# ShudaLi/rgbd_pose_estimation

Measured on AMD Instinct MI355X. Metric: correspondence-residuals/sec, higher is better.
Workload: dtype f32; 1 GPU; configs[1]: 640x480 dense depth, 307200 3D-3D corr, point-to-point GN step (K1 normal eq + host 6x6 solve + SE3 exp) over inlier mask; corr_rank0=307200, global_corr=307200, collective=none, rccl_ranks=0, rccl_verified=False, repeats=1

## Files before the change

### rgbd_pose_estimation_amd/csrc/rpe_normal_eq.hip

```cpp
#include "rpe_residuals.hpp"

namespace rpe {

__global__ void gn_update_probe_kernel(const double* __restrict__ rec, double* __restrict__ pose, double* __restrict__ step_ok,
                                       double rel_floor) {
  __shared__ double s_rec[32];
  __shared__ double s_pose[12];
  if (threadIdx.x < 32) s_rec[threadIdx.x] = rec[threadIdx.x];
  if (threadIdx.x < 12) s_pose[threadIdx.x] = pose[threadIdx.x];
  __syncthreads();
  if (threadIdx.x == 0) {
    double step = 0.0;
    const bool ok = gn_solve_update<0>(s_rec, s_pose, &step, rel_floor);
    step_ok[0] = step; step_ok[1] = ok ? 1.0 : 0.0;
    if (ok) for (int k = 0; k < 12; k++) pose[k] = s_pose[k];
  }
}
hipError_t launch_gn_update_probe(const double* d_rec, double* d_pose, double* d_step_ok, double pivot_floor, hipStream_t s) {
  hipLaunchKernelGGL(gn_update_probe_kernel, dim3(1), dim3(64), 0, s, d_rec, d_pose, d_step_ok, pivot_floor);
  return hipGetLastError();
}

template <class T, int KIND, int BLK, bool MASK, bool WEIGHT, bool CLEAN>
__global__ __launch_bounds__(BLK) void normal_eq_kernel(const T* __restrict__ xw, const T* __restrict__ b, const T* __restrict__ c,
// ... 65 lines not shown
    if (++carried == kShare) { flush_pairs<T, NACC>(carry, acc); carried = 0; }
    a0 = na0; a1 = na1; a2 = na2; b0 = nb0; b1 = nb1; b2 = nb2;
    if (KIND == KIND_P2PLANE) { c0 = nc0; c1 = nc1; c2 = nc2; }
    __builtin_amdgcn_sched_barrier(0);
    pin16(a0); pin16(a1); pin16(a2); pin16(b0); pin16(b1); pin16(b2);
    if (KIND == KIND_P2PLANE) { pin16(c0); pin16(c1); pin16(c2); }
#pragma unroll
    for (int i = 0; i < P; i++) { if (MASK) m[i] = nm[i]; if (WEIGHT) wv[i] = nwv[i]; }
    g = gn;
  }
  if (blockIdx.x == 0 && threadIdx.x == 0 && full * P < n) {
    T vw[3 * P], vb[3 * P], vc[3 * P];
    short lm[P];
    T lwv[P];
    load_group<T>(xw, full, n, vw);
    load_group<T>(b, full, n, vb);
    if (KIND == KIND_P2PLANE) load_group<T>(c, full, n, vc);
    if (MASK) load_scalars<T, short>(mask, full, n, lm, (short)0);
    if (WEIGHT) load_scalars<T, T>(weight, full, n, lwv, T(0));
    pair_group<T, KIND, MASK, WEIGHT, CLEAN, NACC>(pose, vw, vb, vc, lm, lwv, (int)(n - full * P), carry);
    carried = 1;
  }
  if (carried) flush_pairs<T, NACC>(carry, acc);
  RPE_STAMP(1);
  reduce_and_finish<NACC, kNeLd, KIND == KIND_P2P ? 1 : 0, BLK>(acc, fin);
}

template <class T, int KIND, int BLK, bool MASK, bool WEIGHT, int NREG, int AUTO, bool CLEAN>
__global__ __launch_bounds__(BLK) void normal_eq_resident_kernel(const T* __restrict__ xw, const T* __restrict__ b, const T* __restrict__ c,
                             const short* __restrict__ mask, const T* __restrict__ weight, int64_t n,
                             const unsigned long long* __restrict__ ctl, unsigned long long first_tag, int max_iters, Finish fin) {
  constexpr int P = Pk<T>::P;
  constexpr int NACC = KIND == KIND_P2P ? 17 : 29;
  constexpr bool IN_REGS = NREG > 0;
  constexpr int GPT = IN_REGS ? NREG : 1;
  __shared__ double s_pose[12];
  __shared__ int s_go;
  const int64_t full = n / P, groups = (n + P - 1) / P;
  constexpr bool with_solver = AUTO == 2;
  const int workers = (int)gridDim.x;
  const int64_t stride = (int64_t)workers * BLK;
  const int64_t g0 = (int64_t)blockIdx.x * (BLK * GPT) + threadIdx.x;
  T rw[GPT][3 * P], rb[GPT][3 * P], rc[GPT][3 * P];
  short rm[GPT][P];
  T rwv[GPT][P];
  int rpresent[GPT];
#pragma unroll
  for (int r = 0; r < GPT; r++) {
    rpresent[r] = 0;
    const int64_t g = g0 + (int64_t)r * BLK;
    if (IN_REGS && g < groups) {
      load_any_group<T, KIND, MASK, WEIGHT>(xw, b, c, mask, weight, g, full, n, rw[r], rb[r], rc[r], rm[r], rwv[r]);
      rpresent[r] = g < full ? P : (int)(n - full * P);
    }
  }
#ifdef RPE_SOLVER_DEBUG
  if (with_solver && threadIdx.x == 0) __hip_atomic_store(solver_pose_area(fin, workers, NACC) + 32 + blockIdx.x, wall_clock64(), __ATOMIC_RELAXED, __HIP_MEMORY_SCOPE_AGENT);
#endif
  constexpr bool autonomous = AUTO != 0;
  double tol = 0.0;
  if (autonomous) {
    if (threadIdx.x < 12) s_pose[threadIdx.x] = fin.gn_pose[threadIdx.x];
    tol = fin.gn->tol;
    __syncthreads();
  }
  for (int it = 1; it <= max_iters; it++) {
    if (!autonomous && resident_wait_pose<BLK>(ctl, first_tag + (unsigned long long)it, s_pose, &s_go,
        fin.pose_wait_ticks) != 1) return;
    if (with_solver && it > 1 && solver_wait_pose<BLK>(solver_pose_area(fin, workers, NACC), first_tag + (unsigned long long)it, s_pose, &s_go, it == 2 ? kSolverMeetTicks : 200000000ull) != 0) return;
#ifdef RPE_STAMPS
    const bool stamp_it = it == 1000;
    if (stamp_it) RPE_STAMP(0);
#endif
    PoseK<double> pose;
#pragma unroll
    for (int k = 0; k < 9; k++) pose.R[k] = s_pose[k];
#pragma unroll
    for (int k = 0; k < 3; k++) pose.t[k] = s_pose[9 + k];
    double acc[NACC];
#pragma unroll
    for (int k = 0; k < NACC; k++) acc[k] = 0.0;
    if (IN_REGS) {
#pragma unroll
      for (int r = 0; r < GPT; r++)
        if (rpresent[r] > 0) normal_eq_group<T, KIND, MASK, WEIGHT, NACC, CLEAN>(pose, rw[r], rb[r], rc[r], rm[r], rwv[r], rpresent[r], acc);
    } else {
      for (int64_t g = g0; g < groups; g += stride) {
        T vw[3 * P], vb[3 * P], vc[3 * P];
        short mm[P];
        T ww[P];
        load_any_group<T, KIND, MASK, WEIGHT>(xw, b, c, mask, weight, g, full, n, vw, vb, vc, mm, ww);
        normal_eq_group<T, KIND, MASK, WEIGHT, NACC, CLEAN>(pose, vw, vb, vc, mm, ww, g < full ? P : (int)(n - full * P), acc);
      }
    }
#ifdef RPE_STAMPS
    if (stamp_it) RPE_STAMP(1);
#endif
#ifndef RPE_STAMPS
    const bool stamp_it = false;
#endif
    if (with_solver) { solver_send_sums<NACC, BLK>(acc, fin, first_tag + (unsigned long long)it); continue; }
    if (autonomous) {
      if (resident_auto_stage<NACC, BLK>(acc, fin, first_tag + (unsigned long long)it, it, max_iters, tol, s_pose,
          stamp_it) != 0) return;
      continue;
    }
    if (!resident_cross_stage<NACC, BLK>(acc, fin, first_tag + (unsigned long long)it, fin.seq + (unsigned long long)it,
        stamp_it)) return;
  }
}

#ifdef RPE_STAMPS
}
extern "C" int rpe_debug_read_stamps(unsigned long long* out, int nwords) {
  if (nwords > 4096 * 16) nwords = 4096 * 16;
  if (hipDeviceSynchronize() != hipSuccess) return -1;
  if (hipMemcpyFromSymbol(out, HIP_SYMBOL(rpe::g_stamps), (size_t)nwords * 8) != hipSuccess) return -1;
  static unsigned long long zeros[4096 * 16];
  return hipMemcpyToSymbol(HIP_SYMBOL(rpe::g_stamps), zeros, sizeof(zeros)) == hipSuccess ? 0 : -1;
}
namespace rpe {
#endif

template <int MODE>
__global__ __launch_bounds__(64) void chain_finish_kernel(const double* __restrict__ runs, const double* __restrict__ pose_in, GnState* st,
                                                          double rel_floor, double* __restrict__ h_pairs, unsigned long long seq) {
  __shared__ double f_tot[32];
  __shared__ double f_pose[12];
  __shared__ double f_out[16];
  if (threadIdx.x < 12) f_pose[threadIdx.x] = pose_in[threadIdx.x];
  if (threadIdx.x < 32) {
    double t = 0.0;
#pragma unroll
    for (int r = 0; r < kRunSlots; r++) t += runs[r * kRunLd + threadIdx.x];
    f_tot[threadIdx.x] = t;
  }
  __syncthreads();
  if (threadIdx.x == 0) {
    double step = st->step;
    bool ok = st->status == 0;
    if (!st->done) ok = gn_solve_update<MODE>(f_tot, f_pose, &step, rel_floor);
    for (int k = 0; k < 12; k++) f_out[k] = f_pose[k];
    f_out[12] = step; f_out[13] = st->done ? st->cost : record_entry<MODE>(f_tot, 27); f_out[14] = (double)(st->iters + (st->done ? 0 : 1));
    f_out[15] = ok ? 0.0 : 1.0;
  }
  __syncthreads();
  if (threadIdx.x < 16) store_tagged_pair(h_pairs, threadIdx.x, f_out[threadIdx.x], seq);
}
hipError_t launch_chain_finish(int kind, const double* d_runs, const double* d_pose, GnState* d_state, double pivot_floor, double* h_pairs,
                               unsigned long long seq, hipStream_t s) {
  if (kind == KIND_P2P) hipLaunchKernelGGL((chain_finish_kernel<1>), dim3(1), dim3(64), 0, s, d_runs, d_pose, d_state, pivot_floor, h_pairs, seq);
  else hipLaunchKernelGGL((chain_finish_kernel<0>), dim3(1), dim3(64), 0, s, d_runs, d_pose, d_state, pivot_floor, h_pairs, seq);
  return hipGetLastError();
}

template <class T, int KIND, int BLK>
static void normal_eq_launch(const DeviceArrays& A, int flags, const PoseK<double>& pose, const ReduceTarget& rt, hipStream_t s,
                             hipEvent_t ev0, hipEvent_t ev1) {
  const T* xw = (const T*)A.a[0];
  const T* b = (const T*)((KIND == KIND_BEARING || KIND == KIND_REPROJ) ? A.a[2] : A.a[1]);
  const T* c = (const T*)A.a[4];
  const int mod = (KIND == KIND_BEARING || KIND == KIND_REPROJ) ? 0 : 1;
  const short* mask = (flags & F_USE_MASK) ? A.mask[mod] : nullptr;
  const T* weight = (flags & F_USE_WEIGHT) ? (const T*)A.weight[mod] : nullptr;
  const int G = reduce_grid(A.n, Pk<T>::P, rt.max_blocks, BLK);
  const Finish fin = make_finish(rt);
#define RPE_NE_LAUNCH2(M, W, C) RPE_LAUNCH_EV((normal_eq_kernel<T, KIND, BLK, M, W, C>), dim3(G), dim3(BLK), 0, s, ev0, ev1, xw, b, c, mask, weight, A.n, pose, fin)
#define RPE_NE_LAUNCH(M, W) do { if constexpr (sizeof(T) == 4) { if (rt.clean) { RPE_NE_LAUNCH2(M, W, true); break; } } RPE_NE_LAUNCH2(M, W, false); } while (0)
// ... 150 lines not shown
```

### rgbd_pose_estimation_amd/csrc/rpe_reduce.hpp

```cpp
#pragma once
#include "rpe_kernels.h"
#include <cstring>
#include <cstdlib>
#include <algorithm>
#include <hip/hip_ext.h>

namespace rpe {

#ifdef RPE_STAMPS
static __device__ unsigned long long g_stamps[4096 * 16];
#define RPE_STAMP(k)                                                                                             \
  do {                                                                                                           \
    __builtin_amdgcn_sched_barrier(0);                                                                           \
    if (threadIdx.x == 0) {                                                                                      \
      unsigned long long t_;                                                                                     \
      asm volatile("s_memrealtime %0\n\ts_waitcnt lgkmcnt(0)" : "=s"(t_) : : "memory");                          \
      g_stamps[(size_t)blockIdx.x * 16 + (k)] = t_;                                                              \
    }                                                                                                            \
    __builtin_amdgcn_sched_barrier(0);                                                                           \
  } while (0)
#else
#define RPE_STAMP(k) do {} while (0)
#endif

// ... 429 lines not shown
}

template <int NACC, int LD, int BLK, int U>
__device__ __forceinline__ void sum_records(const double* __restrict__ partials, int first, int step, int count, double (*part)[LD],
                                            double* __restrict__ tot) {
  constexpr int RG = BLK / LD;
  const int j = threadIdx.x % LD, rg = threadIdx.x / LD;
  double s = 0.0;
  if (j < NACC) {
    for (int r0 = rg; r0 < count; r0 += RG * U) {
      double v[U];
#pragma unroll
      for (int u = 0; u < U; u++) {
        const int r = r0 + u * RG;
        v[u] = r < count ? __hip_atomic_load(partials + (size_t)(first + r * step) * LD + j, __ATOMIC_RELAXED,
            __HIP_MEMORY_SCOPE_AGENT) : 0.0;
      }
#pragma unroll
      for (int u = 0; u < U; u++) s += v[u];
    }
  }
  part[rg][j] = s;
  __syncthreads();
  if (threadIdx.x < LD) {
    double t = 0.0;
#pragma unroll
    for (int k = 0; k < RG; k++) t += part[k][threadIdx.x];
    tot[threadIdx.x] = threadIdx.x < NACC ? t : 0.0;
  }
}

template <int NACC, int BLK, int CH = 4>
__device__ __forceinline__ bool collect_rows(unsigned long long* __restrict__ gran, int G, int leader, int rows, unsigned long long tag,
                                             double (*part)[NACC], int step = 1,
                                             unsigned long long wait_ticks = 200000000ull) {
  constexpr int RGN = BLK / NACC;
  const int j = threadIdx.x % NACC, r = threadIdx.x / NACC;
  bool lost = false;
  if (CH == 1) {
    if (r >= 1 && r < rows) {
      const unsigned long long* src = gran + 2 * ((size_t)(leader + r * step) * NACC + j);
      const unsigned long long t0 = wall_clock64();
      granule_t q;
      for (unsigned int spins = 1;; spins++) {
        q = load_granule16(src);
        if ((((unsigned long long)q.w << 32) | q.z) == tag) break;
        if ((spins & 63u) == 0 && wall_clock64() - t0 > wait_ticks) { lost = true; break; }
      }
      part[r][j] = __longlong_as_double((long long)(((unsigned long long)q.y << 32) | q.x));
    }
  } else if (r < RGN && r < rows) {
    double sum = r == 0 ? part[0][j] : 0.0;
    const auto rsrc = __builtin_amdgcn_make_buffer_rsrc(reinterpret_cast<void*>(gran), 0, G * NACC * 16, 0x00020000);
    const unsigned long long t0 = wall_clock64();
    for (int k0 = r == 0 ? RGN : r; k0 < rows && !lost; k0 += CH * RGN) {
      granule_t q[CH];
      for (unsigned int spins = 1;; spins++) {
        bool pending = false;
        asm volatile("" ::: "memory");
#pragma unroll
        for (int u = 0; u < CH; u++) {
          const int row = k0 + u * RGN;
          if (row < rows) q[u] = __builtin_amdgcn_raw_buffer_load_b128(rsrc, ((leader + row * step) * NACC + j) * 16, 0, 16);
        }
#pragma unroll
        for (int u = 0; u < CH; u++) {
          const int row = k0 + u * RGN;
          if (row < rows && (((unsigned long long)q[u].w << 32) | q[u].z) != tag) pending = true;
        }
        if (!pending) break;
        if ((spins & 63u) == 0 && wall_clock64() - t0 > wait_ticks) { lost = true; break; }
      }
#pragma unroll
      for (int u = 0; u < CH; u++) {
        const int row = k0 + u * RGN;
        if (row < rows && !lost) sum += __longlong_as_double((long long)(((unsigned long long)q[u].y << 32) | q[u].x));
      }
    }
    part[r][j] = sum;
  }
  return lost;
}

template <int NACC, int RGN>
__device__ __forceinline__ double sum_rows_lane(const double (*part)[NACC], int nr, int j) {
  constexpr int CH = RGN < 16 ? RGN : 16;
  double a = 0.0, b = 0.0;
  for (int k0 = 0; k0 < nr; k0 += CH) {
    double v[CH];
#pragma unroll
    for (int k = 0; k < CH; k++) v[k] = part[k0 + k < RGN ? k0 + k : RGN - 1][j];
#pragma unroll
    for (int k = 0; k < CH; k += 2) {
      a += k0 + k < nr ? v[k] : 0.0;
      if (k + 1 < CH) b += k0 + k + 1 < nr ? v[k + 1] : 0.0;
    }
  }
  return a + b;
}

template <int NACC, int BLK>
__device__ __forceinline__ double sum_rows(const double (*part)[NACC], int nr) {
  constexpr int RGN = BLK / NACC, RB = 6, NB = (RGN + RB - 1) / RB;
  static_assert(NB * NACC <= BLK, "one thread per (block of rows, value)");
  __shared__ double s_blk[NB][NACC];
  const int j = threadIdx.x % NACC, q = threadIdx.x / NACC;
  if (q < NB) {
    double v[RB];
#pragma unroll
    for (int u = 0; u < RB; u++) { const int k = q * RB + u; v[u] = k < nr ? part[k < RGN ? k : 0][j] : 0.0; }
    double t = v[0];
#pragma unroll
    for (int u = 1; u < RB; u++) t += v[u];
    s_blk[q][j] = t;
  }
  __syncthreads();
  double t = 0.0;
  if (threadIdx.x < NACC) {
    t = s_blk[0][threadIdx.x];
#pragma unroll
    for (int b = 1; b < NB; b++) t += s_blk[b][threadIdx.x];
  }
  return t;
}

template <int NACC, int MODE, int BLK>
__device__ __forceinline__ void collect_and_send(const double (*red)[NACC], const Finish& fin) {
  constexpr int NW = BLK / 64;
  constexpr int RGN = BLK / NACC;
  constexpr int kMaxRuns = 512 / NACC > 0 ? 512 / NACC : 1;
  __shared__ double c_part[RGN][NACC];
  unsigned long long* gran = reinterpret_cast<unsigned long long*>(fin.partials);
  const int G = gridDim.x;
  int mult = (G + RGN * 8 - 1) / (RGN * 8);
  if (mult > 4) mult = 4;
  const int mult_cap = (G + RGN * kMaxRuns - 1) / (RGN * kMaxRuns);
  if (mult < mult_cap) mult = mult_cap;
  int R = RGN * mult;
  if (R > fin.rows) R = fin.rows;
  const int S = fin.stride;
  const bool per_xcd = S > 1 && S * NACC <= 512 + NACC && G >= 4 * S && (G + S - 1) / S <= 4 * RGN && (G + S - 1) / S <= fin.rows;
  const int run = per_xcd ? (int)blockIdx.x % S : (int)blockIdx.x / R, leader = per_xcd ? run : run * R, step = per_xcd ? S : 1;
  const int nruns = per_xcd ? S : (G + R - 1) / R;
  if (threadIdx.x < NACC) {
    double own = red[0][threadIdx.x];
#pragma unroll
    for (int w = 1; w < NW; w++) own += red[w][threadIdx.x];
    if ((int)blockIdx.x != leader) store_granule16(gran + 2 * ((size_t)blockIdx.x * NACC + threadIdx.x), own, fin.seq);
    else c_part[0][threadIdx.x] = own;
  }
  RPE_STAMP(4);
  if ((int)blockIdx.x != leader) return;
  const int rows = per_xcd ? (G - run + S - 1) / S : min(R, G - leader);
  const bool lost = collect_rows<NACC, BLK>(gran, G, leader, rows, fin.seq, c_part, step);
  RPE_STAMP(7);
  if (__syncthreads_or(lost)) return;
  RPE_STAMP(8);
  if (fin.out_dev != nullptr) {
    if (threadIdx.x < NACC) fin.out_dev[run * kRunLd + threadIdx.x] = sum_rows_lane<NACC, RGN>(c_part, rows < RGN ? rows : RGN, threadIdx.x);
    if (blockIdx.x == 0) for (int i = nruns * kRunLd + (int)threadIdx.x; i < kRunSlots * kRunLd; i += BLK) fin.out_dev[i] = 0.0;
    return;
  }
  if (threadIdx.x < NACC) store_tagged_pair(fin.out_host, 1 + run * NACC + threadIdx.x,
      sum_rows_lane<NACC, RGN>(c_part, rows < RGN ? rows : RGN, threadIdx.x), fin.seq);
  if (blockIdx.x == 0 && threadIdx.x == 64) {
    const unsigned long long hdr = (unsigned long long)nruns | ((unsigned long long)NACC << 16) | ((unsigned long long)MODE << 24);
    store_tagged_pair(fin.out_host, 0, __longlong_as_double((long long)hdr), fin.seq);
  }
  RPE_STAMP(9);
}

template <int NACC, int LD, int MODE, int BLK, bool GN = true>
__device__ __forceinline__ void reduce_and_finish(double (&acc)[NACC], const Finish& fin) {
  constexpr int NW = BLK / 64;
  constexpr int RG = BLK / LD;
  __shared__ double red[NW][NACC];
  __shared__ double part[RG][LD];
  __shared__ double tot[LD];
  __shared__ int s_last;
  const int lane = threadIdx.x & 63, wave = threadIdx.x >> 6;
  wave_reduce_to<NACC>(acc, red[wave], lane);
  RPE_STAMP(2);
  __syncthreads();
  RPE_STAMP(3);
  if (fin.rows > 0) { collect_and_send<NACC, MODE, BLK>(red, fin); return; }
  const int G = gridDim.x;
  if (G > 1) {
    if (threadIdx.x < NACC) {
      double s = red[0][threadIdx.x];
#pragma unroll
      for (int w = 1; w < NW; w++) s += red[w][threadIdx.x];
      __hip_atomic_store(fin.partials + (size_t)blockIdx.x * LD + threadIdx.x, s, __ATOMIC_RELAXED, __HIP_MEMORY_SCOPE_AGENT);
    }
    asm volatile("s_waitcnt vmcnt(0)" ::: "memory");
    RPE_STAMP(4);
    __syncthreads();
    RPE_STAMP(5);
    const int shard = blockIdx.x & 7;
    const int in_shard = (G - shard + 7) >> 3, shards = G < 8 ? G : 8;
    const int tailv = fin.tail & 3;
    if (tailv != 1) {
      if (threadIdx.x == 0) {
        int last = 0;
        unsigned int* sc = fin.ticket + 32 * shard;
        if (__hip_atomic_fetch_add(sc, 1u, __ATOMIC_RELAXED, __HIP_MEMORY_SCOPE_AGENT) == (unsigned int)in_shard - 1) {
          __hip_atomic_store(sc, 0u, __ATOMIC_RELAXED, __HIP_MEMORY_SCOPE_AGENT);
          unsigned int* top = fin.ticket + 32 * 8;
          if (__hip_atomic_fetch_add(top, 1u, __ATOMIC_RELAXED, __HIP_MEMORY_SCOPE_AGENT) == (unsigned int)shards - 1) {
            __hip_atomic_store(top, 0u, __ATOMIC_RELAXED, __HIP_MEMORY_SCOPE_AGENT);
            last = 1;
          }
        }
        s_last = last;
      }
      RPE_STAMP(6);
      __syncthreads();
      if (!s_last) return;
      RPE_STAMP(7);
      if (tailv == 2) sum_records<NACC, LD, BLK, 16>(fin.partials, 0, 1, G, part, tot);
      else sum_records<NACC, LD, BLK, 8>(fin.partials, 0, 1, G, part, tot);
      RPE_STAMP(8);
    } else {
      if (threadIdx.x == 0) {
        unsigned int* sc = fin.ticket + 32 * shard;
        const int last = __hip_atomic_fetch_add(sc, 1u, __ATOMIC_RELAXED, __HIP_MEMORY_SCOPE_AGENT) == (unsigned int)in_shard - 1;
        if (last) __hip_atomic_store(sc, 0u, __ATOMIC_RELAXED, __HIP_MEMORY_SCOPE_AGENT);
        s_last = last;
      }
      RPE_STAMP(6);
      __syncthreads();
      if (!s_last) return;
      RPE_STAMP(7);
      sum_records<NACC, LD, BLK, 4>(fin.partials, shard, 8, in_shard, part, tot);
      __syncthreads();
      if (threadIdx.x < LD) __hip_atomic_store(fin.partials + (size_t)(G + shard) * LD + threadIdx.x, tot[threadIdx.x],
          __ATOMIC_RELAXED, __HIP_MEMORY_SCOPE_AGENT);
      asm volatile("s_waitcnt vmcnt(0)" ::: "memory");
      __syncthreads();
      RPE_STAMP(8);
// ... 130 lines not shown
```

### rgbd_pose_estimation_amd/csrc/rpe_residuals.hpp

```cpp
#pragma once
#include "rpe_reduce.hpp"

namespace rpe {

template <class C> __device__ __forceinline__ void add_row(const C (&J)[6], C r, C w, C (&s)[29]) {
  int k = 0;
#pragma unroll
  for (int a = 0; a < 6; a++) {
    const C wa = w * J[a];
#pragma unroll
    for (int b = a; b < 6; b++) { s[k] = fma(wa, J[b], s[k]); k++; }
    s[21 + a] = fma(wa, r, s[21 + a]);
  }
  s[27] = fma(w * r, r, s[27]);
}
template <class V> __device__ __forceinline__ void add_row2(const V (&J)[6], V r, V w, V (&s)[29]) {
  int k = 0;
#pragma unroll
  for (int a = 0; a < 6; a++) {
    const V wa = w * J[a];
#pragma unroll
    for (int b = a; b < 6; b++) { s[k] = __builtin_elementwise_fma(wa, J[b], s[k]); k++; }
    s[21 + a] = __builtin_elementwise_fma(wa, r, s[21 + a]);
  }
// ... 158 lines not shown
      V{w[0], w[1]},
                  V{w[0], w[1]}, s);
}


template <class V> __device__ __forceinline__ void p2p_accumulate(V px, V py, V pz, V rx, V ry, V rz, V w, V (&s)[17]) {
  const V wpx = w * px, wpy = w * py, wpz = w * pz;
  const V wrx = w * rx, wry = w * ry, wrz = w * rz;
  s[0] += w;
  s[1] += wpx; s[2] += wpy; s[3] += wpz;
  s[4] = __builtin_elementwise_fma(wpx, px, s[4]); s[5] = __builtin_elementwise_fma(wpx, py, s[5]);
  s[6] = __builtin_elementwise_fma(wpx, pz, s[6]); s[7] = __builtin_elementwise_fma(wpy, py, s[7]);
  s[8] = __builtin_elementwise_fma(wpy, pz, s[8]); s[9] = __builtin_elementwise_fma(wpz, pz, s[9]);
  s[10] += wrx; s[11] += wry; s[12] += wrz;
  s[13] += py * wrz - pz * wry;
  s[14] += pz * wrx - px * wrz;
  s[15] += px * wry - py * wrx;
  s[16] = __builtin_elementwise_fma(wrx, rx, __builtin_elementwise_fma(wry, ry, __builtin_elementwise_fma(wrz, rz, s[16])));
}
template <class C>
__device__ __forceinline__ void p2p_pair(const PoseK<double>& T, const C (&x)[2], const C (&y)[2], const C (&z)[2], const C (&cx)[2],
                                         const C (&cy)[2], const C (&cz)[2], const C (&w)[2], C __attribute__((ext_vector_type(2))) (&s)[17]) {
  typedef C V __attribute__((ext_vector_type(2)));
  C px[2], py[2], pz[2], rx[2], ry[2], rz[2];
#pragma unroll
  for (int e = 0; e < 2; e++) {
    double pxd, pyd, pzd;
    transform<C>(T, x[e], y[e], z[e], pxd, pyd, pzd);
    px[e] = (C)pxd; py[e] = (C)pyd; pz[e] = (C)pzd;
    rx[e] = (C)(pxd - (double)cx[e]); ry[e] = (C)(pyd - (double)cy[e]); rz[e] = (C)(pzd - (double)cz[e]);
  }
  p2p_accumulate<V>(V{px[0], px[1]}, V{py[0], py[1]}, V{pz[0], pz[1]}, V{rx[0], rx[1]}, V{ry[0], ry[1]}, V{rz[0], rz[1]}, V{w[0], w[1]}, s);
}

template <class T, int KIND, bool MASK, bool WEIGHT, bool CLEAN, int NS>
__device__ __forceinline__ void pair_group(const PoseK<double>& pose, const T (&vw)[3 * Pk<T>::P], const T (&vb)[3 * Pk<T>::P],
                                           const T (&vc)[3 * Pk<T>::P], const short (&m)[Pk<T>::P], const T (&wv)[Pk<T>::P],
                                           int npresent, T __attribute__((ext_vector_type(2))) (&s2)[NS]) {
  constexpr int P = Pk<T>::P;
  static_assert(NS == (KIND == KIND_P2P ? 17 : 29), "sums per kind");
  static_assert(KIND == KIND_P2P || KIND == KIND_P2PLANE || KIND == KIND_BEARING || KIND == KIND_REPROJ, "residual kinds");
#pragma unroll
  for (int j = 0; j < P / 2; j++) {
    T x[2], y[2], z[2], bx[2], by[2], bz[2], nx[2], ny[2], nz[2], wi[2];
#pragma unroll
    for (int e = 0; e < 2; e++) {
      const int i = 2 * j + e;
      bx[e] = vb[3 * i]; by[e] = vb[3 * i + 1]; bz[e] = vb[3 * i + 2];
      T w = WEIGHT ? wv[i] : T(1);
      if (MASK) w = m[i] == 1 ? w : T(0);
      if (CLEAN) {
        w = i < npresent ? w : T(0);
        x[e] = vw[3 * i]; y[e] = vw[3 * i + 1]; z[e] = vw[3 * i + 2];
        if (KIND == KIND_P2PLANE) { nx[e] = vc[3 * i]; ny[e] = vc[3 * i + 1]; nz[e] = vc[3 * i + 2]; }
      } else {
        w = (i < npresent && !all_nan(bx[e], by[e], bz[e])) ? w : T(0);
        const bool off = w == T(0);
        x[e] = off ? T(0) : vw[3 * i]; y[e] = off ? T(0) : vw[3 * i + 1];
        z[e] = off ? ((KIND == KIND_BEARING || KIND == KIND_REPROJ) ? T(1) : T(0)) : vw[3 * i + 2];
        bx[e] = off ? T(0) : bx[e]; by[e] = off ? T(0) : by[e]; bz[e] = off ? T(1) : bz[e];
        if (KIND == KIND_P2PLANE) { nx[e] = off ? T(0) : vc[3 * i]; ny[e] = off ? T(0) : vc[3 * i + 1];
            nz[e] = off ? T(0) : vc[3 * i + 2]; }
      }
      wi[e] = w;
    }
    if constexpr (KIND == KIND_P2P) p2p_pair<T>(pose, x, y, z, bx, by, bz, wi, s2);
    else if constexpr (KIND == KIND_P2PLANE) p2plane_pair<T>(pose, x, y, z, bx, by, bz, nx, ny, nz, wi, s2);
    else if constexpr (KIND == KIND_BEARING) bearing_pair<T>(pose, x, y, z, bx, by, bz, wi, s2);
    else {
      reproj_pair<T>(pose, x, y, z, bx, by, bz, wi, s2);
      if (CLEAN) {
        typedef T V __attribute__((ext_vector_type(2)));
        const V all = ((V{x[0], x[1]} + V{y[0], y[1]}) + (V{z[0], z[1]} + V{bx[0], bx[1]})) + (V{by[0], by[1]} + V{bz[0], bz[1]});
        s2[27] = __builtin_elementwise_fma(V{T(0), T(0)}, all, s2[27]);
      }
    }
  }
}
template <class T, int NS>
__device__ __forceinline__ void flush_pairs(T __attribute__((ext_vector_type(2))) (&s2)[NS], double (&acc)[NS]) {
  typedef T V __attribute__((ext_vector_type(2)));
#pragma unroll
  for (int k = 0; k < NS; k++) { acc[k] += (double)(s2[k].x + s2[k].y); s2[k] = V{T(0), T(0)}; }
}

template <class T, int KIND, bool MASK, bool WEIGHT, int NACC, bool CLEAN = false>
__device__ __forceinline__ void normal_eq_group(const PoseK<double>& pose, const T (&vw)[3 * Pk<T>::P], const T (&vb)[3 * Pk<T>::P],
                                                const T (&vc)[3 * Pk<T>::P], const short (&m)[Pk<T>::P], const T (&wv)[Pk<T>::P],
                                                int npresent, double (&acc)[NACC]) {
  typedef T V __attribute__((ext_vector_type(2)));
  V s2[NACC];
#pragma unroll
  for (int k = 0; k < NACC; k++) s2[k] = V{T(0), T(0)};
  pair_group<T, KIND, MASK, WEIGHT, CLEAN, NACC>(pose, vw, vb, vc, m, wv, npresent, s2);
  flush_pairs<T, NACC>(s2, acc);
}
constexpr unsigned long long kResidentStop = 1ull << 63;
template <class T, int KIND, bool MASK, bool WEIGHT>
__device__ __forceinline__ void load_any_group(const T* __restrict__ xw, const T* __restrict__ b, const T* __restrict__ c,
                                               const short* __restrict__ mask, const T* __restrict__ weight, int64_t g, int64_t full,
                                               int64_t n, T (&vw)[3 * Pk<T>::P], T (&vb)[3 * Pk<T>::P], T (&vc)[3 * Pk<T>::P],
                                               short (&m)[Pk<T>::P], T (&wv)[Pk<T>::P]) {
  typedef typename Pk<T>::V V;
  if (g < full) {
    const V* xw4 = reinterpret_cast<const V*>(xw);
    const V* b4 = reinterpret_cast<const V*>(b);
    const V x0 = xw4[3 * g], x1 = xw4[3 * g + 1], x2 = xw4[3 * g + 2];
    const V y0 = b4[3 * g], y1 = b4[3 * g + 1], y2 = b4[3 * g + 2];
    unpack3(x0, x1, x2, vw);
    unpack3(y0, y1, y2, vb);
    if (KIND == KIND_P2PLANE) { const V* c4 = reinterpret_cast<const V*>(c);
        const V z0 = c4[3 * g], z1 = c4[3 * g + 1], z2 = c4[3 * g + 2]; unpack3(z0, z1, z2, vc); }
    if (MASK) load_mask_full(mask, g, m);
    if (WEIGHT) load_weight_full(weight, g, wv);
  } else {
    load_group<T>(xw, g, n, vw);
    load_group<T>(b, g, n, vb);
    if (KIND == KIND_P2PLANE) load_group<T>(c, g, n, vc);
    if (MASK) load_scalars<T, short>(mask, g, n, m, (short)0);
    if (WEIGHT) load_scalars<T, T>(weight, g, n, wv, T(0));
  }
}

constexpr int kAutoMaxRunSums = 1024;
__device__ __forceinline__ int resident_judge_pose(unsigned long long w, unsigned long long want) {
  const unsigned int lo = (unsigned int)w, hi = (unsigned int)(w >> 32);
  const unsigned long long ta = ((unsigned long long)__builtin_amdgcn_readlane(hi, 0) << 32) | __builtin_amdgcn_readlane(lo, 0);
  const unsigned long long tb = ((unsigned long long)__builtin_amdgcn_readlane(hi, 15) << 32) | __builtin_amdgcn_readlane(lo, 15);
  if (ta != tb) return 0;
  const unsigned long long num = ta & ~kResidentStop;
  if (num == want) return (ta & kResidentStop) ? 2 : 1;
  return num > want ? 2 : 0;
}
template <int BLK>
__device__ __forceinline__ int resident_wait_pose(const unsigned long long* __restrict__ ctl, unsigned long long want,
                                                  double* __restrict__ s_pose, int* __restrict__ s_go,
                                                  unsigned long long wait_ticks = 200000000ull) {
  if (threadIdx.x < 64) {
    const int lane = threadIdx.x;
    const unsigned long long t0 = wall_clock64();
    int go = 0;
    unsigned long long w = 0;
    for (;;) {
      if (lane < 16) w = __hip_atomic_load(ctl + lane, __ATOMIC_RELAXED, __HIP_MEMORY_SCOPE_SYSTEM);
      if ((go = resident_judge_pose(w, want)) != 0) break;
      if (wall_clock64() - t0 > wait_ticks) { go = 3; break; }
      __builtin_amdgcn_s_sleep(2);
    }
    if (lane >= 1 && lane <= 12) s_pose[lane - 1] = __longlong_as_double((long long)w);
    if (lane == 0) *s_go = go;
  }
  __syncthreads();
  return *s_go;
}
struct RunShape { int run, row, leader, rows, runs, step; };
__device__ __forceinline__ RunShape run_shape(const Finish& fin, int G) {
  RunShape s;
  const int b = (int)blockIdx.x;
  if (fin.stride > 1) {
    const int S = fin.stride < G ? fin.stride : G;
    s.run = b % S; s.row = b / S; s.leader = s.run; s.rows = (G - s.run + S - 1) / S; s.runs = S; s.step = S;
  } else {
    const int R = fin.rows;
    s.run = b / R; s.leader = s.run * R; s.row = b - s.leader; s.rows = min(R, G - s.leader); s.runs = (G + R - 1) / R; s.step = 1;
  }
  return s;
}
template <int NACC, int BLK>
__device__ __forceinline__ bool resident_cross_own(double own, const Finish& fin, unsigned long long tag, unsigned long long seq, bool stamp_it) {
  constexpr int RGN = BLK / NACC;
  __shared__ double g_part[RGN][NACC];
  unsigned long long* gran = reinterpret_cast<unsigned long long*>(fin.partials);
  const RunShape rs = run_shape(fin, (int)gridDim.x);
  const int run = rs.run, leader = rs.leader;
  if ((int)blockIdx.x != leader) {
    const bool withheld = fin.fault_tag != 0 && tag == fin.fault_tag && blockIdx.x + 1 == gridDim.x;
    if (threadIdx.x < NACC && !withheld) store_granule16(gran + 2 * ((size_t)blockIdx.x * NACC + threadIdx.x), own, tag);
#ifdef RPE_STAMPS
    if (stamp_it) RPE_STAMP(2);
#endif
    return true;
  }
  if (threadIdx.x < NACC) g_part[0][threadIdx.x] = own;
#ifdef RPE_STAMPS
  if (stamp_it) RPE_STAMP(2);
#endif
  const int rows = rs.rows;
  const bool lost = collect_rows<NACC, BLK>(gran, (int)gridDim.x, leader, rows, tag, g_part, rs.step);
#ifdef RPE_STAMPS
  if (stamp_it) RPE_STAMP(3);
#endif
  const bool ok = !__syncthreads_or(lost);
#ifdef RPE_STAMPS
  if (stamp_it) RPE_STAMP(4);
#endif
  if (threadIdx.x < NACC) store_tagged_pair(fin.out_host, run * NACC + threadIdx.x,
      ok ? sum_rows_lane<NACC, RGN>(g_part, rows < RGN ? rows : RGN, threadIdx.x) : __longlong_as_double((long long)kLostMarker), seq);
#ifdef RPE_STAMPS
  if (stamp_it) RPE_STAMP(5);
#endif
  return ok;
}
template <int NACC, int BLK>
__device__ __forceinline__ bool resident_cross_stage(const double (&acc)[NACC], const Finish& fin, unsigned long long tag,
                                                     unsigned long long seq, bool stamp_it) {
  constexpr int NW = BLK / 64;
  __shared__ double g_red[NW][NACC];
  const int lane = threadIdx.x & 63, wave = threadIdx.x >> 6;
  wave_reduce_to<NACC>(acc, g_red[wave], lane);
  __syncthreads();
  double own = 0.0;
  if (threadIdx.x < NACC) {
#pragma unroll
    for (int w = 0; w < NW; w++) own += g_red[w][threadIdx.x];
  }
  return resident_cross_own<NACC, BLK>(own, fin, tag, seq, stamp_it);
}

template <int NACC, int BLK>
__device__ __forceinline__ int resident_auto_stage(const double (&acc)[NACC], const Finish& fin, unsigned long long tag, int it,
                                                   int max_iters, double tol, double* __restrict__ s_pose, bool stamp_it = false) {
  constexpr int NW = BLK / 64;
  constexpr int RGN = BLK / NACC;
  constexpr int MODE = NACC == 17 ? 1 : 0;
  __shared__ double a_red[NW][NACC];
  __shared__ double a_part[RGN][NACC];
  __shared__ double a_runs[kAutoMaxRunSums];
  __shared__ double a_tot[32];
  __shared__ double a_step;
  __shared__ int a_ok;
  const int lane = threadIdx.x & 63, wave = threadIdx.x >> 6;
  const int G = (int)gridDim.x;
  const RunShape rs = run_shape(fin, G);
  const int run = rs.run, leader = rs.leader, runs = rs.runs;
  unsigned long long* gran = reinterpret_cast<unsigned long long*>(fin.partials);
  unsigned long long* rrec = gran + 2 * ((size_t)G * NACC + (size_t)(it & 1) * runs * NACC);
  wave_reduce_to<NACC>(acc, a_red[wave], lane);
  __syncthreads();
  if (threadIdx.x < NACC) {
    double own = 0.0;
#pragma unroll
    for (int w = 0; w < NW; w++) own += a_red[w][threadIdx.x];
    if ((int)blockIdx.x != leader) store_granule16(gran + 2 * ((size_t)blockIdx.x * NACC + threadIdx.x), own, tag);
    else a_part[0][threadIdx.x] = own;
  }
#ifdef RPE_STAMPS
  if (stamp_it) RPE_STAMP(2);
#endif
  bool lost = runs * NACC > kAutoMaxRunSums;
  if (!lost && (int)blockIdx.x == leader) {
    const int rows = rs.rows;
    lost = __syncthreads_or(collect_rows<NACC, BLK>(gran, G, leader, rows, tag, a_part, rs.step));
    if (!lost) {
      const double t = sum_rows<NACC, BLK>(a_part, rows < RGN ? rows : RGN);
      if (threadIdx.x < NACC) { if (G == 1) a_runs[threadIdx.x] = t; else store_granule16(rrec + 2 * ((size_t)run * NACC + threadIdx.x), t, tag); }
    }
  }
#ifdef RPE_STAMPS
  if (stamp_it) RPE_STAMP(3);
#endif
  if (!lost && G > 1) {
    const int total = runs * NACC;
    for (int i = threadIdx.x; i < total; i += BLK) {
      const unsigned long long t0 = wall_clock64();
      granule_t q;
      for (unsigned int spins = 1;; spins++) {
        q = load_granule16(rrec + 2 * (size_t)i);
        if ((((unsigned long long)q.w << 32) | q.z) == tag) break;
        if ((spins & 63u) == 0 && wall_clock64() - t0 > 200000000ull) { lost = true; break; }
      }
      a_runs[i] = __longlong_as_double((long long)(((unsigned long long)q.y << 32) | q.x));
    }
  }
  lost = __syncthreads_or(lost);
#ifdef RPE_STAMPS
  if (stamp_it) RPE_STAMP(4);
#endif
  if (threadIdx.x < 64) {
    if (!lost) {
      double t = 0.0;
      if (threadIdx.x < NACC) for (int r = 0; r < runs; r++) t += a_runs[r * NACC + threadIdx.x];
      if (threadIdx.x < 32) a_tot[threadIdx.x] = threadIdx.x < NACC ? t : 0.0;
    }
    __builtin_amdgcn_fence(__ATOMIC_RELEASE, "wavefront");
    __builtin_amdgcn_wave_barrier();
    __builtin_amdgcn_fence(__ATOMIC_ACQUIRE, "wavefront");
#ifdef RPE_STAMPS
    if (stamp_it) RPE_STAMP(5);
#endif
    if (threadIdx.x == 0) {
      double step = 0.0;
      a_ok = !lost && gn_solve_update<MODE>(a_tot, s_pose, &step, fin.pivot_floor) ? 1 : 0;
      a_step = step;
    }
  }
  __syncthreads();
#ifdef RPE_STAMPS
  if (stamp_it) RPE_STAMP(6);
#endif
  const bool ok = a_ok != 0;
  const bool done = !ok || a_step < tol || it >= max_iters;
  if (done && blockIdx.x == 0 && threadIdx.x == 0 && fin.out_host) {
    for (int k = 0; k < 12; k++) __hip_atomic_store(fin.out_host + k, s_pose[k], __ATOMIC_RELAXED, __HIP_MEMORY_SCOPE_SYSTEM);
    __hip_atomic_store(fin.out_host + 12, a_step, __ATOMIC_RELAXED, __HIP_MEMORY_SCOPE_SYSTEM);
    __hip_atomic_store(fin.out_host + 13, lost ? 0.0 : record_entry<MODE>(a_tot, 27), __ATOMIC_RELAXED, __HIP_MEMORY_SCOPE_SYSTEM);
    __hip_atomic_store(fin.out_host + 14, (double)it, __ATOMIC_RELAXED, __HIP_MEMORY_SCOPE_SYSTEM);
    __hip_atomic_store(fin.out_host + 15, ok ? 0.0 : (lost ? 2.0 : 1.0), __ATOMIC_RELAXED, __HIP_MEMORY_SCOPE_SYSTEM);
    __hip_atomic_store(fin.out_host + 16, lost ? 0.0 : record_entry<MODE>(a_tot, 28), __ATOMIC_RELAXED, __HIP_MEMORY_SCOPE_SYSTEM);
    asm volatile("s_waitcnt vmcnt(0)" ::: "memory");
    __hip_atomic_store(reinterpret_cast<unsigned long long*>(fin.out_host + 32), fin.seq, __ATOMIC_RELAXED, __HIP_MEMORY_SCOPE_SYSTEM);
  }
  return lost ? 2 : (done ? 1 : 0);
}

constexpr int kSolverPoseGranules = 14;
constexpr unsigned long long kSolverMeetTicks = 25000000ull;
__device__ __forceinline__ unsigned long long* solver_pose_area(const Finish& fin, int workers, int nacc) {
  return reinterpret_cast<unsigned long long*>(fin.partials) + 2 * ((size_t)(workers + 8) * nacc);
}
template <int BLK>
__device__ __forceinline__ int solver_wait_pose(const unsigned long long* __restrict__ area, unsigned long long want, double* __restrict__ s_pose,
                                                int* __restrict__ s_go, unsigned long long wait_ticks = 200000000ull) {
  if (threadIdx.x < 64) {
    const int lane = threadIdx.x;
    const unsigned long long t0 = wall_clock64();
    granule_t q = {};
    int go = -1;
    for (unsigned int spins = 1;; spins++) {
      bool have = true;
      if (lane < kSolverPoseGranules) {
        q = load_granule16(area + 2 * (size_t)lane);
        have = (((unsigned long long)q.w << 32) | q.z) == want;
      }
      if (__builtin_amdgcn_ballot_w64(!have) == 0) { go = 0; break; }
      if ((spins & 63u) == 0 && wall_clock64() - t0 > wait_ticks) { go = 3; break; }
      __builtin_amdgcn_s_sleep(1);
    }
    const double v = __longlong_as_double((long long)(((unsigned long long)q.y << 32) | q.x));
    if (lane < 12) s_pose[lane] = v;
    if (lane == 13) *s_go = go == 3 ? 3 : (int)v;
  }
  __syncthreads();
  return *s_go;
}
template <int NACC, int BLK>
__device__ __forceinline__ void solver_send_sums(const double (&acc)[NACC], const Finish& fin, unsigned long long tag) {
  constexpr int NW = BLK / 64;
  __shared__ double w_red[NW][NACC];
  const int lane = threadIdx.x & 63, wave = threadIdx.x >> 6;
  unsigned long long* gran = reinterpret_cast<unsigned long long*>(fin.partials);
  wave_reduce_to<NACC>(acc, w_red[wave], lane);
  __syncthreads();
  if (threadIdx.x < NACC) {
    double own = 0.0;
#pragma unroll
    for (int w = 0; w < NW; w++) own += w_red[w][threadIdx.x];
    store_granule16(gran + 2 * ((size_t)blockIdx.x * NACC + threadIdx.x), own, tag);
  }
  __syncthreads();
}
template <int NACC, int BLK>
__device__ __forceinline__ void solver_loop(const Finish& fin, int workers, unsigned long long first_tag, int max_iters) {
  constexpr int RGN = BLK / NACC;
  constexpr int MODE = NACC == 17 ? 1 : 0;
  __shared__ double v_part[RGN][NACC];
  __shared__ double v_tot[32];
  __shared__ double v_pose[12];
  __shared__ double v_step;
  __shared__ int v_code;
  unsigned long long* gran = reinterpret_cast<unsigned long long*>(fin.partials);
  unsigned long long* area = solver_pose_area(fin, workers, NACC);
#ifdef RPE_SOLVER_DEBUG
  const unsigned long long dbg_start = wall_clock64();
#endif
  if (threadIdx.x < 12) v_pose[threadIdx.x] = fin.gn_pose[threadIdx.x];
  const double tol = fin.gn->tol;
  __syncthreads();
  for (int it = 1; it <= max_iters; it++) {
    const unsigned long long tag = first_tag + (unsigned long long)it;
    if (threadIdx.x < NACC) v_part[0][threadIdx.x] = 0.0;
    __syncthreads();
    bool lost = collect_rows<NACC, BLK, 12>(gran, workers, -1, workers + 1, tag, v_part, 1, it <= 2 ? kSolverMeetTicks : 200000000ull);
    lost = __syncthreads_or(lost);
    if (lost && threadIdx.x == 0 && fin.out_host) {
      int missing = 0, lo = workers, hi = -1;
      for (int w = 0; w < workers; w++) {
        const granule_t q = load_granule16(gran + 2 * ((size_t)w * NACC + NACC - 1));
        if ((((unsigned long long)q.w << 32) | q.z) != tag) { missing++; lo = w < lo ? w : lo; hi = w; }
      }
#ifdef RPE_SOLVER_DEBUG
      {
        unsigned long long mn = ~0ull, mx = 0; int started = 0;
        for (int w = 0; w < workers; w++) {
          const unsigned long long v = __hip_atomic_load(area + 32 + w, __ATOMIC_RELAXED, __HIP_MEMORY_SCOPE_AGENT);
          if (v > dbg_start - 100000000ull) { started++; mn = v < mn ? v : mn; mx = v > mx ? v : mx; }
        }
        __hip_atomic_store(fin.out_host + 20, (double)started, __ATOMIC_RELAXED, __HIP_MEMORY_SCOPE_SYSTEM);
        __hip_atomic_store(fin.out_host + 21, started ? ((double)mn - (double)dbg_start) * 0.01 : -1.0, __ATOMIC_RELAXED, __HIP_MEMORY_SCOPE_SYSTEM);
        __hip_atomic_store(fin.out_host + 22, started ? ((double)mx - (double)dbg_start) * 0.01 : -1.0, __ATOMIC_RELAXED, __HIP_MEMORY_SCOPE_SYSTEM);
        __hip_atomic_store(fin.out_host + 23, ((double)wall_clock64() - (double)dbg_start) * 0.01, __ATOMIC_RELAXED, __HIP_MEMORY_SCOPE_SYSTEM);
      }
#endif
      __hip_atomic_store(fin.out_host + 17, (double)missing, __ATOMIC_RELAXED, __HIP_MEMORY_SCOPE_SYSTEM);
      __hip_atomic_store(fin.out_host + 18, (double)lo, __ATOMIC_RELAXED, __HIP_MEMORY_SCOPE_SYSTEM);
      __hip_atomic_store(fin.out_host + 19, (double)hi, __ATOMIC_RELAXED, __HIP_MEMORY_SCOPE_SYSTEM);
    }
    const double t = sum_rows<NACC, BLK>(v_part, workers + 1 < RGN ? workers + 1 : RGN);
    if (threadIdx.x < 64) {
      if (threadIdx.x < 32) v_tot[threadIdx.x] = threadIdx.x < NACC ? t : 0.0;
      __builtin_amdgcn_fence(__ATOMIC_RELEASE, "wavefront");
      __builtin_amdgcn_wave_barrier();
      __builtin_amdgcn_fence(__ATOMIC_ACQUIRE, "wavefront");
      if (threadIdx.x == 0) {
        double step = 0.0;
        const bool ok = !lost && gn_solve_update<MODE>(v_tot, v_pose, &step, fin.pivot_floor);
        v_step = step;
        v_code = !ok ? 2 : ((step < tol || it >= max_iters) ? 1 : 0);
      }
      __builtin_amdgcn_fence(__ATOMIC_RELEASE, "wavefront");
      __builtin_amdgcn_wave_barrier();
      __builtin_amdgcn_fence(__ATOMIC_ACQUIRE, "wavefront");
      const int lane = threadIdx.x;
      if (lane == 0 && v_code != 0 && fin.out_host) {
        const bool ok = v_code == 1;
        for (int k = 0; k < 12; k++) __hip_atomic_store(fin.out_host + k, v_pose[k], __ATOMIC_RELAXED, __HIP_MEMORY_SCOPE_SYSTEM);
        __hip_atomic_store(fin.out_host + 12, v_step, __ATOMIC_RELAXED, __HIP_MEMORY_SCOPE_SYSTEM);
        __hip_atomic_store(fin.out_host + 13, lost ? 0.0 : record_entry<MODE>(v_tot, 27), __ATOMIC_RELAXED, __HIP_MEMORY_SCOPE_SYSTEM);
        __hip_atomic_store(fin.out_host + 14, (double)it, __ATOMIC_RELAXED, __HIP_MEMORY_SCOPE_SYSTEM);
        __hip_atomic_store(fin.out_host + 15, ok ? 0.0 : (lost ? 2.0 : 1.0), __ATOMIC_RELAXED, __HIP_MEMORY_SCOPE_SYSTEM);
        __hip_atomic_store(fin.out_host + 16, lost ? 0.0 : record_entry<MODE>(v_tot, 28), __ATOMIC_RELAXED, __HIP_MEMORY_SCOPE_SYSTEM);
        asm volatile("s_waitcnt vmcnt(0)" ::: "memory");
        __hip_atomic_store(reinterpret_cast<unsigned long long*>(fin.out_host + 32), fin.seq, __ATOMIC_RELAXED, __HIP_MEMORY_SCOPE_SYSTEM);
        asm volatile("s_waitcnt vmcnt(0)" ::: "memory");
      }
      __builtin_amdgcn_fence(__ATOMIC_RELEASE, "wavefront");
      __builtin_amdgcn_wave_barrier();
      if (lane < kSolverPoseGranules) {
        const double v = lane < 12 ? v_pose[lane] : (lane == 12 ? v_step : (double)v_code);
        store_granule16(area + 2 * (size_t)lane, v, tag + 1);
      }
    }
    __syncthreads();
    if (v_code != 0) return;
  }
}
static inline bool auto_solver_grid(int workers, int cap) {
  static const int env = getenv("RPE_AUTO_SOLVER") ? atoi(getenv("RPE_AUTO_SOLVER")) : 1;
  static const int env_min = getenv("RPE_AUTO_SOLVER_MIN") ? atoi(getenv("RPE_AUTO_SOLVER_MIN")) : 32;
  return env != 0 && workers >= env_min && workers + 1 <= cap;
}

static inline int resident_block() { return 512; }
constexpr int kResidentGroupsPerThread = 2;

}
```

Before: 46.99 billion correspondence-residuals/s.

## Use paired f32 accumulation in register path and ballot-based block any-reduction

```diff
diff --git a/rgbd_pose_estimation_amd/csrc/rpe_normal_eq.hip b/rgbd_pose_estimation_amd/csrc/rpe_normal_eq.hip
--- a/rgbd_pose_estimation_amd/csrc/rpe_normal_eq.hip
+++ b/rgbd_pose_estimation_amd/csrc/rpe_normal_eq.hip
@@ -171,8 +171,16 @@
     for (int k = 0; k < NACC; k++) acc[k] = 0.0;
     if (IN_REGS) {
 #pragma unroll
-      for (int r = 0; r < GPT; r++)
-        if (rpresent[r] > 0) normal_eq_group<T, KIND, MASK, WEIGHT, NACC, CLEAN>(pose, rw[r], rb[r], rc[r], rm[r], rwv[r], rpresent[r], acc);
+      for (int r = 0; r < GPT; r++) {
+        if (rpresent[r] > 0) {
+          typedef T V2 __attribute__((ext_vector_type(2)));
+          V2 s2[NACC];
+#pragma unroll
+          for (int k = 0; k < NACC; k++) s2[k] = V2{T(0), T(0)};
+          pair_group<T, KIND, MASK, WEIGHT, CLEAN, NACC>(pose, rw[r], rb[r], rc[r], rm[r], rwv[r], rpresent[r], s2);
+          if (r == 0) widen_pairs<T, NACC, true>(s2, acc); else widen_pairs<T, NACC, false>(s2, acc);
+        }
+      }
     } else {
       for (int64_t g = g0; g < groups; g += stride) {
         T vw[3 * P], vb[3 * P], vc[3 * P];
diff --git a/rgbd_pose_estimation_amd/csrc/rpe_reduce.hpp b/rgbd_pose_estimation_amd/csrc/rpe_reduce.hpp
--- a/rgbd_pose_estimation_amd/csrc/rpe_reduce.hpp
+++ b/rgbd_pose_estimation_amd/csrc/rpe_reduce.hpp
@@ -535,6 +535,19 @@
   return lost;
 }
 
+template <int BLK>
+__device__ __forceinline__ bool barrier_any(bool mine, unsigned int* __restrict__ flags) {
+  static_assert(BLK % 64 == 0, "whole waves");
+  constexpr int NW = BLK / 64;
+  const bool wave_any = __builtin_amdgcn_ballot_w64(mine) != 0;
+  if ((threadIdx.x & 63) == 0) flags[threadIdx.x >> 6] = wave_any ? 1u : 0u;
+  __syncthreads();
+  unsigned int any = 0;
+#pragma unroll
+  for (int w = 0; w < NW; w++) any |= flags[w];
+  return __builtin_amdgcn_readfirstlane(any) != 0;
+}
+
 template <int NACC, int RGN>
 __device__ __forceinline__ double sum_rows_lane(const double (*part)[NACC], int nr, int j) {
   constexpr int CH = RGN < 16 ? RGN : 16;
@@ -583,6 +596,7 @@
   constexpr int RGN = BLK / NACC;
   constexpr int kMaxRuns = 512 / NACC > 0 ? 512 / NACC : 1;
   __shared__ double c_part[RGN][NACC];
+  __shared__ unsigned int c_lost[NW];
   unsigned long long* gran = reinterpret_cast<unsigned long long*>(fin.partials);
   const int G = gridDim.x;
   int mult = (G + RGN * 8 - 1) / (RGN * 8);
@@ -607,7 +621,7 @@
   const int rows = per_xcd ? (G - run + S - 1) / S : min(R, G - leader);
   const bool lost = collect_rows<NACC, BLK>(gran, G, leader, rows, fin.seq, c_part, step);
   RPE_STAMP(7);
-  if (__syncthreads_or(lost)) return;
+  if (barrier_any<BLK>(lost, c_lost)) return;
   RPE_STAMP(8);
   if (fin.out_dev != nullptr) {
     if (threadIdx.x < NACC) fin.out_dev[run * kRunLd + threadIdx.x] = sum_rows_lane<NACC, RGN>(c_part, rows < RGN ? rows : RGN, threadIdx.x);
diff --git a/rgbd_pose_estimation_amd/csrc/rpe_residuals.hpp b/rgbd_pose_estimation_amd/csrc/rpe_residuals.hpp
--- a/rgbd_pose_estimation_amd/csrc/rpe_residuals.hpp
+++ b/rgbd_pose_estimation_amd/csrc/rpe_residuals.hpp
@@ -264,6 +264,15 @@
   typedef T V __attribute__((ext_vector_type(2)));
 #pragma unroll
   for (int k = 0; k < NS; k++) { acc[k] += (double)(s2[k].x + s2[k].y); s2[k] = V{T(0), T(0)}; }
+}
+template <class T, int NS, bool FIRST>
+__device__ __forceinline__ void widen_pairs(const T __attribute__((ext_vector_type(2))) (&s2)[NS], double (&acc)[NS]) {
+#pragma unroll
+  for (int k = 0; k < NS; k++) {
+    T t = s2[k].x + s2[k].y;
+    asm("" : "+v"(t));
+    acc[k] = FIRST ? (double)t : acc[k] + (double)t;
+  }
 }
 
 template <class T, int KIND, bool MASK, bool WEIGHT, int NACC, bool CLEAN = false>
@@ -352,6 +361,7 @@
 __device__ __forceinline__ bool resident_cross_own(double own, const Finish& fin, unsigned long long tag, unsigned long long seq, bool stamp_it) {
   constexpr int RGN = BLK / NACC;
   __shared__ double g_part[RGN][NACC];
+  __shared__ unsigned int g_lost[BLK / 64];
   unsigned long long* gran = reinterpret_cast<unsigned long long*>(fin.partials);
   const RunShape rs = run_shape(fin, (int)gridDim.x);
   const int run = rs.run, leader = rs.leader;
@@ -372,7 +382,7 @@
 #ifdef RPE_STAMPS
   if (stamp_it) RPE_STAMP(3);
 #endif
-  const bool ok = !__syncthreads_or(lost);
+  const bool ok = !barrier_any<BLK>(lost, g_lost);
 #ifdef RPE_STAMPS
   if (stamp_it) RPE_STAMP(4);
 #endif
@@ -411,6 +421,7 @@
   __shared__ double a_tot[32];
   __shared__ double a_step;
   __shared__ int a_ok;
+  __shared__ unsigned int a_lost_rows[NW], a_lost_runs[NW];
   const int lane = threadIdx.x & 63, wave = threadIdx.x >> 6;
   const int G = (int)gridDim.x;
   const RunShape rs = run_shape(fin, G);
@@ -432,7 +443,7 @@
   bool lost = runs * NACC > kAutoMaxRunSums;
   if (!lost && (int)blockIdx.x == leader) {
     const int rows = rs.rows;
-    lost = __syncthreads_or(collect_rows<NACC, BLK>(gran, G, leader, rows, tag, a_part, rs.step));
+    lost = barrier_any<BLK>(collect_rows<NACC, BLK>(gran, G, leader, rows, tag, a_part, rs.step), a_lost_rows);
     if (!lost) {
       const double t = sum_rows<NACC, BLK>(a_part, rows < RGN ? rows : RGN);
       if (threadIdx.x < NACC) { if (G == 1) a_runs[threadIdx.x] = t; else store_granule16(rrec + 2 * ((size_t)run * NACC + threadIdx.x), t, tag); }
@@ -454,7 +465,7 @@
       a_runs[i] = __longlong_as_double((long long)(((unsigned long long)q.y << 32) | q.x));
     }
   }
-  lost = __syncthreads_or(lost);
+  lost = barrier_any<BLK>(lost, a_lost_runs);
 #ifdef RPE_STAMPS
   if (stamp_it) RPE_STAMP(4);
 #endif
@@ -550,6 +561,7 @@
   __shared__ double v_pose[12];
   __shared__ double v_step;
   __shared__ int v_code;
+  __shared__ unsigned int v_lost[BLK / 64];
   unsigned long long* gran = reinterpret_cast<unsigned long long*>(fin.partials);
   unsigned long long* area = solver_pose_area(fin, workers, NACC);
 #ifdef RPE_SOLVER_DEBUG
@@ -563,7 +575,7 @@
     if (threadIdx.x < NACC) v_part[0][threadIdx.x] = 0.0;
     __syncthreads();
     bool lost = collect_rows<NACC, BLK, 12>(gran, workers, -1, workers + 1, tag, v_part, 1, it <= 2 ? kSolverMeetTicks : 200000000ull);
-    lost = __syncthreads_or(lost);
+    lost = barrier_any<BLK>(lost, v_lost);
     if (lost && threadIdx.x == 0 && fin.out_host) {
       int missing = 0, lo = workers, hi = -1;
       for (int w = 0; w < workers; w++) {
```

Result: slower. 46.33 billion correspondence-residuals/s (-1.4%).
